# openai/jukebox

Measured on NVIDIA H100. Metric: top_prior_tokens_per_sec, higher is better.
Workload: dtype fp16

## Files before the change

### jukebox_b200/csrc/decode_engine.cu

```cuda
#include "engine.cuh"
#include <cooperative_groups.h>
#include <vector>
#include <algorithm>
#include <string.h>
#include <stdlib.h>
#include <math.h>

using namespace jk;

#ifndef JK_MMA_ALL_WARPS
#define JK_MMA_ALL_WARPS 1
#endif
#ifndef JK_QKV_POLL_BATCH
#define JK_QKV_POLL_BATCH 1
#endif
#ifndef JK_SKIP_FOREIGN_WAIT
#define JK_SKIP_FOREIGN_WAIT 1
#endif
#ifndef JK_LOGITS_MMA
#define JK_LOGITS_MMA 1
#endif
#ifndef JK_ATTN_LL_MERGE
#define JK_ATTN_LL_MERGE 1
#endif

namespace {

constexpr int kConsumers = 256;
constexpr int kThreads = 384;
constexpr int kSlotBytes = 16384;
constexpr int kMaxSlots = 12;
constexpr int kHeaderBytes = 8192;
constexpr int kLogitKT = 1024;
constexpr int kLogitRowsPerChunk = 4;
constexpr int kLogitRowsPerPass = 16;
constexpr int kMaxSplit = 4;
constexpr int kProfSlots = 1024;
// ... 31 lines not shown
    int slot;
    uint32_t phase;
    __device__ __forceinline__ static int nslot() { return sm_E()->nslot; }
    __device__ __forceinline__ uint64_t* full() const { return sm_full() + slot; }
    __device__ __forceinline__ uint64_t* empty() const { return sm_empty() + slot; }
    __device__ __forceinline__ uint8_t* data() const {
        const EngineDev* E = sm_E();
        return jk_smem + kHeaderBytes + E->uni_bytes + E->kvpre_bytes + slot * kSlotBytes;
    }
    __device__ __forceinline__ void advance() {
        if (++slot == nslot()) { slot = 0; phase ^= 1u; }
    }
};

#define STAMP(E_, slot_, i_)                                                                \
    do {                                                                                    \
        if (blockIdx.x == 0 && threadIdx.x == 0 && (E_)->prof_on && (slot_) < kProfSlots)      \
            (E_)->prof2[(size_t)(slot_) * 8 + (i_)] = clock64();                             \
    } while (0)

__device__ __forceinline__ void consumer_sync() { asm volatile("bar.sync 1, 256;" ::: "memory"); }

__device__ __host__ __forceinline__ int kpc_of(int ncg) { return ncg == 1 ? 64 : ncg == 2 ? 32 : ncg <= 4 ? 16 : 8; }

#define JK_ST_LL "st.relaxed.gpu.global"
__device__ __forceinline__ void ll_st(unsigned long long* p, uint32_t data, uint32_t flag) {
    const unsigned long long v = ((unsigned long long)flag << 32) | data;
    asm volatile(JK_ST_LL ".u64 [%0], %1;" ::"l"(p), "l"(v) : "memory");
}
__device__ __forceinline__ ulonglong2 ll_ld2(const unsigned long long* p) {
    ulonglong2 v;
    asm volatile("ld.relaxed.gpu.global.v2.u64 {%0,%1}, [%2];" : "=l"(v.x), "=l"(v.y) : "l"(p) : "memory");
    return v;
}
__device__ __forceinline__ unsigned long long ll_ld1(const unsigned long long* p) {
    unsigned long long v;
    asm volatile("ld.relaxed.gpu.global.u64 %0, [%1];" : "=l"(v) : "l"(p) : "memory");
    return v;
}
__constant__ int jk_nowait;
__device__ __forceinline__ bool ll_ok(unsigned long long w, uint32_t flag) { return ((uint32_t)(w >> 32) == flag) | (jk_nowait != 0); }
__device__ __forceinline__ void spin_guard(unsigned& spins) {
    if (++spins > (1u << 24)) __trap();
}
__device__ __forceinline__ uint32_t ll_wait1(const unsigned long long* p, uint32_t flag) {
    unsigned spins = 0;
    unsigned long long w = ll_ld1(p);
    while (!ll_ok(w, flag)) { spin_guard(spins); w = ll_ld1(p); }
    return (uint32_t)w;
}
__device__ __forceinline__ unsigned long long wait_stat_word(const long long* p, int G) {
    unsigned spins = 0;
    unsigned long long w = ll_ld1(reinterpret_cast<const unsigned long long*>(p));
    while ((int)(w >> kCntShift) != G && !jk_nowait) { spin_guard(spins); w = ll_ld1(reinterpret_cast<const unsigned long long*>(p)); }
    return w;
}

__device__ __forceinline__ float quick_gelu_f(float x) {
    const float z = h2f_round(1.702f * x);
    const float s = h2f_round(1.0f / (1.0f + expf(-z)));
    return x * s;
}

__device__ __forceinline__ long long fx_sum(float x) { return __float2ll_rn(x * 65536.0f); }
__device__ __forceinline__ long long fx_sq(float x) { return __float2ll_rn(fminf(x * x, 16777216.0f) * 16384.0f); }
__device__ __forceinline__ void red_add_u64(long long* p, unsigned long long v) {
    atomicAdd(reinterpret_cast<unsigned long long*>(p), v);
}
__device__ __forceinline__ long long* sm_sfx() { return reinterpret_cast<long long*>(sm_uni() + kRedBytes); }

__device__ __forceinline__ void publish_stats(long long* ln_out, int B, int ppc) {
    const int tid = threadIdx.x;
// ... 167 lines not shown

struct LogitsRec {
    float* lg_out;
    long long lg_bs;
    const float* lb;
    long long lb_bs;
    unsigned long long* xp;
    ushort2 cols;
};
__device__ __forceinline__ LogitsRec* sm_lrec() { return reinterpret_cast<LogitsRec*>(jk_smem + 7744); }

__device__ __noinline__ Ring gemm_phase(Ring ring, int B, int epi_, int l, int pslot_, uint32_t fl) {
    const EngineDev* E = sm_E();
    GemmArgs g;
    {
        const LayerDev& LD = *sm_layer(l);
        const ushort2* cl = reinterpret_cast<const ushort2*>(jk_smem + 1024 + 256 * (l & 1) + 128);
        const int W = E->W, S = E->S, M = E->M;
        long long* lnb = E->lnacc + (size_t)(2 * l) * 512;
        g.epi = epi_; g.pslot = pslot_; g.flag_in = fl; g.flag_out = fl;
        g.gamma = nullptr; g.beta = nullptr; g.ln_in = nullptr; g.ln_out = nullptr; g.ln = 0;
        g.lg_out = nullptr; g.lg_bs = 0; g.lb = nullptr; g.lb_bs = 0;
        if (epi_ == EPI_QKV) {
            g.in = E->ll_h; g.out = E->ll_qkv; g.xp = E->xp[0]; g.K = W; g.N = (LD.attn_func == 6) ? S : 3 * S;
            g.g0 = cl[0].x; g.ncg = cl[0].y; g.ln = 1; g.gamma = LD.ln0_g; g.beta = LD.ln0_b; g.bias = LD.b_qkv;
            g.ln_in = lnb; g.kind = 0; g.kin = W;
        } else if (epi_ == EPI_PROJ) {
            g.in = E->ll_a; g.out = E->ll_x1; g.xp = E->xp[1]; g.K = S; g.N = W; g.g0 = cl[1].x; g.ncg = cl[1].y;
            g.bias = LD.b_o; g.ln_out = lnb + 512; g.kind = 1; g.kin = S;
        } else if (epi_ == EPI_FC) {
            g.in = E->ll_x1; g.out = E->ll_g; g.xp = E->xp[2]; g.K = W; g.N = M; g.g0 = cl[2].x; g.ncg = cl[2].y;
            g.ln = 1; g.gamma = LD.ln1_g; g.beta = LD.ln1_b; g.bias = LD.b_1; g.ln_in = lnb + 512; g.kind = 0; g.kin = W;
        } else if (epi_ == EPI_PROJ2) {
            g.in = E->ll_g; g.out = E->ll_h; g.xp = E->xp[3]; g.K = M; g.N = W; g.g0 = cl[3].x; g.ncg = cl[3].y;
            g.bias = LD.b_2; g.ln_out = lnb + 1024; g.flag_out = fl + 1; g.kind = 2; g.kin = M;
        } else {
            const LogitsRec* lr = sm_lrec();
            g.in = E->ll_h; g.out = nullptr; g.xp = lr->xp; g.K = 2 * W; g.N = E->bins; g.g0 = lr->cols.x; g.ncg = lr->cols.y;
            g.bias = nullptr; g.kind = 2; g.kin = W; g.flag_out = 0;
            g.lg_out = lr->lg_out; g.lg_bs = lr->lg_bs; g.lb = lr->lb; g.lb_bs = lr->lb_bs;
        }
    }
    uint8_t* uni = sm_uni();
    const int tid = threadIdx.x, warp = tid >> 5, lane = tid & 31;
    const int KS = E->KS, ksh = E->ks_shift, c = blockIdx.x, rank = c & (KS - 1);
    const int ncg = g.ncg, nc = ncg * 8;
    const int ppc = (nc >> 1) >> ksh;
    const bool residual = (g.epi == EPI_PROJ || g.epi == EPI_PROJ2);
// ... 67 lines not shown
    STAMP(E, g.pslot, 2);
#if JK_MMA_ALL_WARPS
    const int nwarp = in_order ? min(8, nslots_phase) : min(8, nkk);
#else
    const int nwarp = min(8, (nkk + kpc - 1) >> (31 - __clz(kpc)));
#endif
    float* red = reinterpret_cast<float*>(uni);
    const int ncp = ((nc + 31) & ~31) + 8;
    unsigned long long* xp_unit = g.xp + (size_t)(c - rank) * 16 * kXpCols;
    {
        consumer_sync();
        if (warp < nwarp) {
            const int r0 = lane >> 2, c0 = (lane & 3) * 2;
#pragma unroll
            for (int j = 0; j < 8; ++j) {
                if (j < ncg) {
                    float* d = red + (size_t)(warp * 16) * ncp + j * 8 + c0;
                    *reinterpret_cast<float2*>(d + r0 * ncp) = make_float2(acc[j][0], acc[j][1]);
                    *reinterpret_cast<float2*>(d + (r0 + 8) * ncp) = make_float2(acc[j][2], acc[j][3]);
                }
            }
        }
        consumer_sync();
        if (KS > 1 && lane < (nc >> 1)) {
#pragma unroll 1
            for (int b = warp; b < B; b += 8) {
                float s0 = 0.f, s1 = 0.f;
                for (int w = 0; w < nwarp; ++w) {
                    const float2 v = *reinterpret_cast<const float2*>(red + (size_t)(w * 16 + b) * ncp + 2 * lane);
                    s0 += v.x; s1 += v.y;
                }
                unsigned long long* dst = xp_unit + ((size_t)rank * 16 + b) * kXpCols + 2 * lane;
                const unsigned long long fl = (unsigned long long)g.flag_in << 32;
                asm volatile(JK_ST_LL ".v2.u64 [%0], {%1,%2};" ::"l"(dst), "l"(fl | __float_as_uint(s0)),
                             "l"(fl | __float_as_uint(s1)) : "memory");
            }
        }
    }
    STAMP(E, g.pslot, 3);
    float2* res = sm_res();
    long long* sfx = sm_sfx();
    const bool two_rows = ppc <= 16;
    const int pl = two_rows ? (lane & 15) : lane;
    const int b_first = two_rows ? 2 * warp + (lane >> 4) : warp, b_step = two_rows ? 16 : 8;
    if (pl < ppc) {
        const int pr = rank * ppc + pl;
        const int gc = g.g0 * 8 + 2 * pr;
        const float2 bias = g.bias ? *reinterpret_cast<const float2*>(g.bias + gc) : make_float2(0.f, 0.f);
#pragma unroll 1
        for (int b = b_first; b < B; b += b_step) {
            float s0 = 0.f, s1 = 0.f;
            if (KS == 1) {
                for (int w = 0; w < nwarp; ++w) {
                    const float2 v = *reinterpret_cast<const float2*>(red + (size_t)(w * 16 + b) * ncp + 2 * pr);
                    s0 += v.x; s1 += v.y;
                }
            } else {
                ulonglong2 v[4];
                unsigned spins = 0;
                bool again;
                do {
                    again = false;
#pragma unroll
                    for (int q = 0; q < 4; ++q)
                        if (q < KS) v[q] = ll_ld2(xp_unit + ((size_t)q * 16 + b) * kXpCols + 2 * pr);
#pragma unroll
                    for (int q = 0; q < 4; ++q)
                        if (q < KS) again |= !(ll_ok(v[q].x, g.flag_in) && ll_ok(v[q].y, g.flag_in));
                    if (again) spin_guard(spins);
                } while (again);
#pragma unroll
                for (int q = 0; q < 4; ++q)
                    if (q < KS) { s0 += __uint_as_float((uint32_t)v[q].x); s1 += __uint_as_float((uint32_t)v[q].y); }
            }
            if (epi == EPI_LOGITS) {
                float* lo_ = g.lg_out + (size_t)b * g.lg_bs + gc;
                const float* lb_ = g.lb ? g.lb + (size_t)b * g.lb_bs + gc : nullptr;
                if (gc < N) lo_[0] = s0 + (lb_ ? lb_[0] : 0.f);
                if (gc + 1 < N) lo_[1] = s1 + (lb_ ? lb_[1] : 0.f);
                continue;
            }
            const float y0 = h2f_round(s0 + bias.x), y1 = h2f_round(s1 + bias.y);
            __half2 o;
            if (epi == EPI_QKV) {
                o = __floats2half2_rn(y0, y1);
            } else if (epi == EPI_FC) {
                o = __floats2half2_rn(quick_gelu_f(y0), quick_gelu_f(y1));
            } else {
                const float2 base = res[b * 32 + pl];
                const float o0 = h2f_round(base.x + y0), o1 = h2f_round(base.y + y1);
                res[b * 32 + pl] = make_float2(o0, o1);
                o = __floats2half2_rn(o0, o1);
                sfx[b * 32 + pl] = fx_sum(o0) + fx_sum(o1);
                sfx[1024 + b * 32 + pl] = fx_sq(o0) + fx_sq(o1);
            }
            ll_st(g.out + (size_t)b * (N >> 1) + (gc >> 1), *reinterpret_cast<const uint32_t*>(&o), g.flag_out);
        }
    }
    STAMP(E, g.pslot, 4);
    if (residual) publish_stats(g.ln_out, B, ppc);
    else consumer_sync();
    return ring;
}

struct AttnGeom {
    int R;
    int base;
    int cur;
    int wrow;
// ... 108 lines not shown
#pragma unroll
        for (int q = 0; q < 4; ++q) {
            const bool on = q < ns;
            m[q] = on ? __ldcg(p0 + (size_t)q * st) : -INFINITY;
            l[q] = on ? __ldcg(p0 + (size_t)q * st + 1) : 0.f;
            v[q] = (on && d < dh) ? __ldcg(reinterpret_cast<const float2*>(p0 + (size_t)q * st + 2 + d)) : make_float2(0.f, 0.f);
        }
        float M = -INFINITY;
#pragma unroll
        for (int q = 0; q < 4; ++q) M = fmaxf(M, m[q]);
        float Lsum = 0.f, o0 = 0.f, o1 = 0.f;
#pragma unroll
        for (int q = 0; q < 4; ++q) {
            if (q < ns) {
                const float w = expf(m[q] - M);
                Lsum += l[q] * w; o0 += v[q].x * w; o1 += v[q].y * w;
            }
        }
        if (d < dh) attn_out_pair(E, b, h, d, o0 / Lsum, o1 / Lsum, flag);
    }
}

__device__ __noinline__ void attn_item(const LayerDev& LD_ref, int b, int h, int s, int ns,
                                       const AttnGeom G, int pslot, uint32_t flag, int pre) {
    const EngineDev* E = sm_E();
    uint8_t* uni = sm_uni();
    float* stats = sm_stats();
    const LayerDev LD = LD_ref;
    const int tid = threadIdx.x, lane = tid & 31, warp = tid >> 5;
    const int dh = E->dh, dhp = E->dh_pad, S = E->S;
    const int nvec = dhp >> 3, npair = dhp >> 4;
    const int swz = (nvec & 7) ? 0 : 7;
    const int RC = E->RC;
    const int tileB = RC * dhp * 2;
    const uint32_t regU = smem_u32(uni), regX = smem_u32(jk_smem + kHeaderBytes + E->uni_bytes);
    const uint32_t regA = pre ? regX : regU, regB = pre ? regU : regX;
    __half* qh = reinterpret_cast<__half*>(uni + 2 * tileB);
    __half* kn = qh + dhp;
    __half* vn = kn + dhp;
    float* sc = reinterpret_cast<float*>(uni + 2 * tileB + 3 * dhp * 2);
    const int qkv_words = ((LD.attn_func == 6) ? S : 3 * S) >> 1;
    const unsigned long long* qrow = E->ll_qkv + (size_t)b * qkv_words + ((h * dh) >> 1);
    const size_t cbase = ((size_t)(b * E->H + h)) * LD.rows;
    const bool last_part = (s == ns - 1);
    const int R = G.R;
    const int ncache = R - ((R > 0 && G.cur) ? 1 : 0);
    const int i0 = div_small(ncache * s, ns), i1 = div_small(ncache * (s + 1), ns);
    const __half* kbase = LD.kc + (cbase + G.base) * dhp;
    const __half* vbase = LD.vc + (cbase + G.base) * dhp;
    const int trows = RC - 1;
    const int ntiles = max(1, (i1 - i0 + trows - 1) / trows);

    auto issue_tile = [&](int ti) {
        const int r0 = i0 + ti * trows, nr = max(0, min(trows, i1 - r0));
        const uint32_t kd = (ti & 1) ? regB : regA, vd = kd + tileB;
        kv_copy_tile(kd, vd, kbase + (size_t)r0 * dhp, vbase + (size_t)r0 * dhp, nr, dhp, swz);
    };
    STAMP(E, pslot, 0);
    if (R > 0 && !pre) issue_tile(0);
    {
        const int hw = dhp >> 1, dw = dh >> 1;
        const int nsel = (LD.attn_func == 6) ? 1 : 3;
#if JK_QKV_POLL_BATCH
        const int total = nsel * hw;
        unsigned long long wv[3];
        const unsigned long long* wp[3];
#pragma unroll
        for (int j = 0; j < 3; ++j) {
            const int i = tid + j * kConsumers;
            const int sel = (i >= hw) + (i >= 2 * hw), wd = i - sel * hw;
            wp[j] = (i < total && wd < dw) ? qrow + (size_t)sel * (S >> 1) + wd : nullptr;
            if (wp[j]) wv[j] = ll_ld1(wp[j]);
        }
        unsigned spins = 0;
        for (;;) {
            bool again = false;
#pragma unroll
            for (int j = 0; j < 3; ++j)
                if (wp[j] && !ll_ok(wv[j], flag)) { wv[j] = ll_ld1(wp[j]); again = true; }
            if (!again) break;
            spin_guard(spins);
        }
#pragma unroll
        for (int j = 0; j < 3; ++j) {
            const int i = tid + j * kConsumers;
            if (i < total) reinterpret_cast<uint32_t*>(qh)[i] = wp[j] ? (uint32_t)wv[j] : 0u;
        }
#else
        for (int i = tid; i < nsel * hw; i += kConsumers) {
            const int sel = i / hw, wd = i - sel * hw;
            uint32_t v = 0u;
            if (wd < dw) v = ll_wait1(qrow + (size_t)sel * (S >> 1) + wd, flag);
            reinterpret_cast<uint32_t*>(qh)[sel * hw + wd] = v;
        }
#endif
    }
    consumer_sync();
    if (G.wrow >= 0 && last_part) {
        for (int i = tid; i < dh; i += kConsumers) {
            LD.kc[(cbase + G.wrow) * dhp + i] = kn[i];
            LD.vc[(cbase + G.wrow) * dhp + i] = vn[i];
        }
    }
    if (R == 0) {
        if (2 * tid < dh) attn_out_pair(E, b, h, 2 * tid, 0.f, 0.f, flag);
        return;
    }

    float m_run = -INFINITY, l_run = 0.f;
    float* osm = sc + 64;
    const uint32_t qh_s = smem_u32(qh);
#pragma unroll 1
    for (int ti = 0; ti < ntiles; ++ti) {
        if (ti + 1 < ntiles) {
            issue_tile(ti + 1);
            asm volatile("cp.async.wait_group 1;" ::: "memory");
        } else {
            asm volatile("cp.async.wait_group 0;" ::: "memory");
// ... 151 lines not shown
            attn_out_pair(E, b, h, d, o0 / Lsum, o1 / Lsum, flag);
        }
        STAMP(E, pslot, 6);
        return;
    }
#endif
    const int item = b * E->H + h;
    if (tid == 0) {
        float* part = E->part + ((size_t)(item * kMaxSplit + s)) * (dhp + 2);
        part[0] = m_run; part[1] = l_run;
    }
    consumer_sync();
    if (tid == 0) {
        unsigned ticket;
        asm volatile("atom.acq_rel.gpu.global.add.u32 %0, [%1], 1;" : "=r"(ticket) : "l"(E->acnt + item) : "memory");
        stats[48] = (ticket == (unsigned)(ns - 1)) ? 1.f : 0.f;
        if (ticket == (unsigned)(ns - 1)) E->acnt[item] = 0u;
    }
    consumer_sync();
    if (stats[48] != 0.f) attn_merge(item, ns, b, h, flag);
    STAMP(E, pslot, 6);
}

__device__ __noinline__ int attn_prefetch(const LayerDev& LD_ref, int B, int c, int t, int pm, int pd, int gmax) {
    const EngineDev* E = sm_E();
    if (!E->kv_prefetch) return 0;
    const LayerDev LD = LD_ref;
    const AttnGeom G = attn_geom(E, LD, t, pm, pd);
    if (G.R == 0) return 0;
    const int ncache = G.R - (G.cur ? 1 : 0);
    const int ns = attn_nsplit(E, gmax, ncache);
    if (c >= B * E->H * ns) return 0;
    const int bh = div_small(c, ns), s = c - bh * ns, b = bh / E->H, h = bh - b * E->H;
    const int dhp = E->dh_pad, nvec = dhp >> 3, RC = E->RC;
    const int swz = (nvec & 7) ? 0 : 7;
    const int i0 = div_small(ncache * s, ns), i1 = div_small(ncache * (s + 1), ns);
    const int nr = max(0, min(RC - 1, i1 - i0));
    const size_t cbase = ((size_t)(b * E->H + h)) * LD.rows;
    const uint32_t kd = smem_u32(jk_smem + kHeaderBytes + E->uni_bytes), vd = kd + RC * dhp * 2;
    kv_copy_tile(kd, vd, LD.kc + (cbase + G.base + i0) * dhp, LD.vc + (cbase + G.base + i0) * dhp, nr, dhp, swz);
    return 1;
}

__device__ __noinline__ void producer_loop(const EngineDev* E, Ring ring, int do_logits, int c) {
    if ((threadIdx.x & 31) != 0) return;
    const uint8_t* src = E->streams + (size_t)c * E->stream_stride;
// ... 293 lines not shown
                const float2 pe = *reinterpret_cast<const float2*>(E->pos_emb + (size_t)launch_pos() * E->W + col);
                x.x += pe.x; x.y += pe.y;
                if (A.x_cond) {
                    const float2 xc = *reinterpret_cast<const float2*>(A.x_cond + ((size_t)b * A.x_cond_len + (A.x_cond_len > 1 ? launch_pos() : 0)) * E->W + col);
                    x.x += xc.x; x.y += xc.y;
                }
            }
            const __half2 hh = __floats2half2_rn(x.x, x.y);
            const float2 hv = __half22float2(hh);
            res[b * 32 + pl] = hv;
            sfx[b * 32 + pl] = fx_sum(hv.x) + fx_sum(hv.y);
            sfx[1024 + b * 32 + pl] = fx_sq(hv.x) + fx_sq(hv.y);
            ll_st(E->ll_h + (((size_t)b * E->W + col) >> 1), *reinterpret_cast<const uint32_t*>(&hh), launch_fbase() + 1);
        }
        publish_stats(LN_BLOCK(0), B, ppc);
    }
    PHASE_DONE();

#pragma unroll 1
    for (int l = 0; l < E->depth; ++l) {
        const LayerDev& LD = *sm_layer(l);
        const uint32_t fl = launch_fbase() + (uint32_t)l + 1;
        const int pre = attn_prefetch(LD, B, c, launch_pos(), PM, PD, GMAX);
        if (l == 1) PROF3(0, 0);
        ring = gemm_phase(ring, B, EPI_QKV, l, (int)nph, fl);
        if (l == 1) PROF3(0, 1);
        if (l > 0) CLEAR_AFTER(2 * l - 1, 2 * l);
        if (l + 1 < E->depth) {
#if JK_ASYNC_RECORD
            if (tid < (int)(sizeof(LayerDev) / 4))
                asm volatile("cp.async.ca.shared.global [%0], [%1], 4;" ::"r"(smem_u32(jk_smem + 1024 + 256 * ((l + 1) & 1) + 4 * tid)),
                             "l"(reinterpret_cast<const uint32_t*>(&Eg->layer[l + 1]) + tid) : "memory");
            if (tid >= 32 && tid < 36)
                asm volatile("cp.async.ca.shared.global [%0], [%1], 4;" ::"r"(smem_u32(jk_smem + 1024 + 256 * ((l + 1) & 1) + 128 + 4 * (tid - 32))),
                             "l"(reinterpret_cast<const uint32_t*>(E->cols + ((size_t)cta_unit() * E->depth + l + 1) * 4) + (tid - 32)) : "memory");
            asm volatile("cp.async.commit_group;" ::: "memory");
#else
            if (tid < (int)(sizeof(LayerDev) / 4))
                reinterpret_cast<uint32_t*>(jk_smem + 1024 + 256 * ((l + 1) & 1))[tid] =
                    reinterpret_cast<const uint32_t*>(&Eg->layer[l + 1])[tid];
            if (tid >= 32 && tid < 36)
                reinterpret_cast<uint32_t*>(jk_smem + 1024 + 256 * ((l + 1) & 1) + 128)[tid - 32] =
                    reinterpret_cast<const uint32_t*>(E->cols + ((size_t)cta_unit() * E->depth + l + 1) * 4)[tid - 32];
#endif
        }
        PHASE_DONE();
        if (l == 1) PROF3(1, 0);
        {
            const AttnGeom geo = attn_geom(E, LD, launch_pos(), PM, PD);
            const int ns = attn_nsplit(E, GMAX, geo.R - ((geo.R > 0 && geo.cur) ? 1 : 0));
            for (int it = c; it < B * E->H * ns; it += E->G) {
                const int bh = div_small(it, ns), s = it - bh * ns, ib = bh / E->H;
                attn_item(LD, ib, bh - ib * E->H, s, ns, geo, (int)nph, fl, pre && it == c);
                consumer_sync();
            }
        }
        if (l == 1) PROF3(1, 1);
        PHASE_DONE();
        if (l == 1) PROF3(2, 0);
        ring = gemm_phase(ring, B, EPI_PROJ, l, (int)nph, fl);
        if (l == 1) PROF3(2, 1);
        PHASE_DONE();
        if (l == 1) PROF3(3, 0);
        ring = gemm_phase(ring, B, EPI_FC, l, (int)nph, fl);
        if (l == 1) PROF3(3, 1);
        CLEAR_AFTER(2 * l, 2 * l + 1);
        PHASE_DONE();
        if (l == 1) PROF3(4, 0);
#if JK_ASYNC_RECORD
        asm volatile("cp.async.wait_group 0;" ::: "memory");
#endif
        ring = gemm_phase(ring, B, EPI_PROJ2, l, (int)nph, fl);
        if (l == 1) PROF3(4, 1);
        PHASE_DONE();
    }
    if (A.h_out) {
// ... 136 lines not shown
    for (int i = threadIdx.y; i < 32; i += blockDim.y) {
        const int n = n0 + i, k = k0 + threadIdx.x;
        if (n < N && k < K) dst[(size_t)n * K + k] = tile[threadIdx.x][i];
    }
}

__global__ void enc_kv_scatter_kernel(const __half* __restrict__ y, __half* kc, __half* vc, int rows_total, int E_dims,
                                      int S, int H, int dh, int dhp) {
    const size_t i = (size_t)blockIdx.x * blockDim.x + threadIdx.x;
    if (i >= (size_t)rows_total * 2 * S) return;
    const int r = (int)(i / (2 * S)), cidx = (int)(i % (2 * S));
    const int b = r / E_dims, e = r % E_dims;
    const int which = cidx / S, cs = cidx % S;
    const int h = cs / dh, d = cs % dh;
    __half* dst = which ? vc : kc;
    dst[(((size_t)(b * H + h)) * E_dims + e) * dhp + d] = y[i];
}

}

namespace {

struct Layout {
    size_t off_dev, off_cols, off_goff, off_lrow, off_streams, off_small, off_cache, off_h, off_x1, off_qkv, off_a, off_g, off_xp[4], off_part, off_acnt, off_prof, off_prof2, off_prof3, off_lnacc, off_encx, off_ency, off_wt, off_pf, off_sync, total;
    int KS, U;
    size_t wt_per_layer;
    int pf_len, pf_rows;
    size_t stream_stride;
    std::vector<ushort2> cols;
    std::vector<uint32_t> goff;
    std::vector<int> lrow;
    int lg_on, lg_np;
    std::vector<size_t> cache_off;
    std::vector<size_t> cache_bytes;
    std::vector<int> cache_rows;
    size_t small_per_layer;
    int dh, dh_pad, bc, prime_pad, uni_bytes, kvpre_bytes, kv_prefetch, nslot, smem_bytes, RC;
};

inline size_t align_up(size_t v, size_t a) { return (v + a - 1) / a * a; }

int cache_rows_for(const jk_prior_config& c, int af, int bc, int prime_pad) {
    switch (af) {
        case 0: return c.n_ctx;
        case 1: return bc;
        case 2: return c.n_ctx;
        case 3: return 2 * bc;
        case 6: return c.encoder_dims;
        case 7: return prime_pad;
    }
    return -1;
}

int compute_layout(const jk_prior_config& c, int G, Layout& L) {
// ... 42 lines not shown
            JK_REQUIRE(base + (extra ? 1 : 0) <= 8, "n_out %d too wide for %d units (max 64 columns per unit)", Ns[gi], U);
            std::vector<int> n(U, base);
            if (gi == 1 || gi == 3) {
                for (int i = 0; i < extra; ++i) n[i] += 1;
            } else {
                const unsigned long long chunk = (unsigned long long)(Ks[gi] / KS / 16) * 256ull;
                for (int i = 0; i < extra; ++i) {
                    int best = -1;
                    for (int u = 0; u < U; ++u)
                        if (n[u] < 8 && (best < 0 || cum[u] + n[u] * chunk < cum[best] + n[best] * chunk)) best = u;
                    n[best] += 1;
                }
            }
            int g0 = 0;
            for (int u = 0; u < U; ++u) {
                L.cols[((size_t)u * depth + l) * 4 + gi] = make_ushort2((unsigned short)g0, (unsigned short)n[u]);
                for (int r = 0; r < KS; ++r)
                    L.goff[((size_t)(u * KS + r) * depth + l) * 4 + gi] = (uint32_t)(cum[u] / 16);
                cum[u] += (unsigned long long)n[u] * (Ks[gi] / KS / 16) * 256ull;
                g0 += n[u];
            }
        }
    }
    L.lg_on = 0; L.lg_np = 0;
    {
        const int groups = (c.bins + 7) / 8;
        const int Kp = 2 * c.width;
        const int np = ((groups + U - 1) / U + 7) / 8;
        const bool ok = c.bins > 0 && KS >= 2 && (Kp / 16) % KS == 0 && c.width % (Kp / KS) == 0 &&
                        (size_t)16 * (Kp / KS + 8) * 2 <= (size_t)65536 && np <= 4 && !getenv("JK_NO_LOGITS_MMA");
        if (ok) {
            L.lg_on = 1; L.lg_np = np;
            L.cols.resize((size_t)U * depth * 4 + (size_t)np * U, make_ushort2(0, 0));
            L.goff.resize((size_t)G * depth * 4 + (size_t)np * G, 0);
            const int base = groups / U, extra = groups % U;
            std::vector<int> n(U, base);
            for (int i = 0; i < U; ++i) order[i] = i;
            std::stable_sort(order.begin(), order.end(), [&](int a, int b) { return cum[a] < cum[b]; });
            for (int i = 0; i < extra; ++i) n[order[i]] += 1;
            std::vector<int> g0(U, 0);
            for (int u = 1; u < U; ++u) g0[u] = g0[u - 1] + n[u - 1];
            for (int p = 0; p < np; ++p) {
                for (int u = 0; u < U; ++u) {
                    const int k = std::max(0, std::min(8, n[u] - 8 * p));
                    L.cols[(size_t)U * depth * 4 + (size_t)p * U + u] = make_ushort2((unsigned short)(g0[u] + 8 * p), (unsigned short)k);
                    for (int r = 0; r < KS; ++r) L.goff[(size_t)G * depth * 4 + (size_t)p * G + u * KS + r] = (uint32_t)(cum[u] / 16);
// ... 18 lines not shown
        uni = std::max(uni, (size_t)16 * kLogitKT * 4);
        uni = std::max(uni, (size_t)kRedBytes + 2 * 1024 * 8);
        const size_t kv_stage = (size_t)2 * RC * L.dh_pad * 2;
        size_t attn = kv_stage + (size_t)3 * L.dh_pad * 2 + 64 * 4 + (size_t)L.dh_pad * 4 + 64;
        uni = std::max(uni, attn);
        L.uni_bytes = (int)align_up(uni, 1024);
        L.kvpre_bytes = (int)align_up(kv_stage, 1024);
        nslot = (max_smem - kHeaderBytes - L.uni_bytes - L.kvpre_bytes) / kSlotBytes;
        if (nslot >= 4 || RC <= 16) break;
    }
    L.RC = RC;
    L.kv_prefetch = 0;
    nslot = std::min(nslot, kMaxSlots);
    JK_REQUIRE(nslot >= 2, "not enough shared memory for the weight ring (uni %d bytes)", L.uni_bytes);
    L.nslot = nslot;
    L.smem_bytes = kHeaderBytes + L.uni_bytes + L.kvpre_bytes + nslot * kSlotBytes;
    JK_REQUIRE((size_t)kHeaderBytes + (size_t)16 * (Kmax + 8) * 2 <= (size_t)L.smem_bytes, "A tile exceeds shared memory");

    size_t off = 0;
    L.off_dev = off; off = align_up(off + sizeof(EngineDev), 256);
    L.off_cols = off; off = align_up(off + L.cols.size() * sizeof(ushort2), 256);
    L.off_goff = off; off = align_up(off + L.goff.size() * 4, 256);
    L.off_lrow = off; off = align_up(off + L.lrow.size() * 4, 256);
    L.off_streams = off; off = align_up(off + (size_t)G * L.stream_stride, 256);
    L.small_per_layer = align_up((size_t)(3 * c.n_state + c.width + c.mlp_width + c.width + 4 * c.width) * 4, 256);
    L.off_small = off; off += L.small_per_layer * depth;
    for (int l = 0; l < depth; ++l)
        if (c.attn_func[l] == 6) off = align_up(off + (size_t)c.width * 2 * c.n_state * 2 + 2 * c.n_state * 4 + 512, 256);
    L.off_cache = off;
    L.cache_off.resize(depth); L.cache_bytes.resize(depth); L.cache_rows.resize(depth);
    for (int l = 0; l < depth; ++l) {
        int rows = cache_rows_for(c, c.attn_func[l], L.bc, L.prime_pad);
        L.cache_rows[l] = rows;
        size_t bytes = align_up((size_t)c.max_batch * c.heads * rows * L.dh_pad * 2, 256);
        L.cache_off[l] = off; L.cache_bytes[l] = bytes;
        off += 2 * bytes;
    }
    L.off_h = off;   off = align_up(off + (size_t)16 * c.width * 4, 256);
    L.off_x1 = off;  off = align_up(off + (size_t)16 * c.width * 4, 256);
    L.off_qkv = off; off = align_up(off + (size_t)16 * 3 * c.n_state * 4, 256);
    L.off_a = off;   off = align_up(off + (size_t)16 * c.n_state * 4, 256);
    L.off_g = off;   off = align_up(off + (size_t)16 * c.mlp_width * 4, 256);
    for (int gi = 0; gi < 4; ++gi) { L.off_xp[gi] = off; off = align_up(off + (size_t)G * 16 * kXpCols * 8, 256); }
    L.off_part = off; off = align_up(off + (size_t)c.max_batch * c.heads * kMaxSplit * (L.dh_pad + 2) * 8, 256);
    L.off_acnt = off; off = align_up(off + (size_t)c.max_batch * c.heads * 4, 256);
    L.off_prof = off; off = align_up(off + (size_t)kProfSlots * 8, 256);
    L.off_prof2 = off; off = align_up(off + (size_t)kProfSlots * 8 * 8, 256);
    L.off_prof3 = off; off = align_up(off + (size_t)5 * 256 * 2 * 8, 256);
    L.off_lnacc = off; off = align_up(off + (size_t)(2 * depth + 1) * 512 * 8, 256);
    {
        bool any6 = false;
        for (int l = 0; l < depth; ++l) any6 = any6 || (c.attn_func[l] == 6);
        L.off_encx = off; if (any6) off = align_up(off + (size_t)c.max_batch * c.encoder_dims * c.width * 2, 1024);
        L.off_ency = off; if (any6) off = align_up(off + (size_t)c.max_batch * c.encoder_dims * 2 * c.n_state * 2, 1024);
    }
    {
        auto k_ok = [](int k) { return k >= 64 && k % 8 == 0; };
        const bool ok = k_ok(c.width) && k_ok(c.n_state) && k_ok(c.mlp_width) && !getenv("JK_NO_PREFILL");
        int cap = c.n_ctx;
        if (const char* e = getenv("JK_PREFILL_MAX")) cap = std::max(2, std::min(cap, atoi(e)));
        L.pf_len = ok ? cap : 0;
        L.pf_rows = c.max_batch * L.pf_len;
        L.wt_per_layer = align_up((size_t)(3 * c.n_state * c.width + c.width * c.n_state + 2 * c.mlp_width * c.width) * 2, 1024);
// ... 75 lines not shown
    E.W = cfg->width; E.S = cfg->n_state; E.M = cfg->mlp_width; E.H = cfg->heads; E.dh = L.dh; E.dh_pad = L.dh_pad;
    E.L = cfg->n_ctx; E.blocks = cfg->blocks; E.bc = L.bc; E.bins = cfg->bins; E.prime_pad = L.prime_pad;
    E.enc_dims = cfg->encoder_dims; E.Bmax = cfg->max_batch; E.add_cond_after = cfg->add_cond_after;
    E.depth = cfg->depth; E.G = G; E.KS = L.KS; E.ks_shift = L.KS == 4 ? 2 : L.KS == 2 ? 1 : 0; E.U = L.U; E.RC = L.RC; E.nslot = L.nslot; E.uni_bytes = L.uni_bytes; E.kvpre_bytes = L.kvpre_bytes; E.small_bytes = (int)L.small_per_layer; E.prof_on = getenv("JK_PROFILE") ? 1 : 0;
    E.kv_prefetch = getenv("JK_KV_PREFETCH") ? atoi(getenv("JK_KV_PREFETCH")) : 1;
    {
        const int nowait = getenv("JK_NOWAIT") ? atoi(getenv("JK_NOWAIT")) : 0;
        JK_CHECK_CUDA(cudaMemcpyToSymbol(jk_nowait, &nowait, sizeof(int)));
    }
    {
        double sc = 1.0 / sqrt(sqrt((double)L.dh));
        E.scale2 = (float)(sc * sc);
    }
    E.cols = (const ushort2*)(A + L.off_cols);
    p->d_cols = (ushort2*)(A + L.off_cols);
    p->d_goff = (uint32_t*)(A + L.off_goff);
    E.lrow0 = (const int*)(A + L.off_lrow);
    E.lg_on = L.lg_on; p->lg_on = L.lg_on;
    E.lg_np = L.lg_np; p->lg_np = L.lg_np;
    E.lg_cols = (const ushort2*)(A + L.off_cols) + (size_t)L.U * cfg->depth * 4;
    E.lg_goff = (const uint32_t*)(A + L.off_goff) + (size_t)G * cfg->depth * 4;
    E.streams = A + L.off_streams; E.stream_stride = L.stream_stride;
    E.ll_h = (unsigned long long*)(A + L.off_h); E.ll_x1 = (unsigned long long*)(A + L.off_x1);
    E.ll_qkv = (unsigned long long*)(A + L.off_qkv); E.ll_a = (unsigned long long*)(A + L.off_a);
    E.ll_g = (unsigned long long*)(A + L.off_g);
    for (int gi = 0; gi < 4; ++gi) E.xp[gi] = (unsigned long long*)(A + L.off_xp[gi]);
    E.part = (float*)(A + L.off_part);
    E.acnt = (unsigned*)(A + L.off_acnt); E.prof = (unsigned long long*)(A + L.off_prof);
    E.lnacc = (long long*)(A + L.off_lnacc);
    E.prof2 = (long long*)(A + L.off_prof2);
    E.prof3 = (unsigned long long*)(A + L.off_prof3);
    E.sync = (unsigned*)(A + L.off_sync); E.t = (int*)(E.sync + 96);
    size_t enc_off = L.off_small + L.small_per_layer * cfg->depth;
    for (int i = 0; i < 4; ++i) { p->bias_ptr[i].resize(cfg->depth); p->ln_ptr[i].resize(cfg->depth); }
    p->enc_w.assign(cfg->depth, nullptr); p->enc_b.assign(cfg->depth, nullptr);
    for (int l = 0; l < cfg->depth; ++l) {
        LayerDev& LD = E.layer[l];
        LD.attn_func = cfg->attn_func[l];
        LD.rows = L.cache_rows[l];
        LD.kc = (__half*)(A + L.cache_off[l]);
        LD.vc = (__half*)(A + L.cache_off[l] + L.cache_bytes[l]);
        float* s = (float*)(A + L.off_small + L.small_per_layer * l);
        p->bias_ptr[0][l] = s; s += 3 * cfg->n_state;
        p->bias_ptr[1][l] = s; s += cfg->width;
        p->bias_ptr[2][l] = s; s += cfg->mlp_width;
        p->bias_ptr[3][l] = s; s += cfg->width;
        for (int i = 0; i < 4; ++i) { p->ln_ptr[i][l] = s; s += cfg->width; }
// ... 14 lines not shown
    p->pf_rows = L.pf_rows; p->pf_len = L.pf_len;
    for (int i = 0; i < 4; ++i) p->wt[i].assign(cfg->depth, nullptr);
    if (L.pf_rows) {
        for (int l = 0; l < cfg->depth; ++l) {
            __half* w = (__half*)(A + L.off_wt + L.wt_per_layer * l);
            p->wt[0][l] = w; w += (size_t)3 * cfg->n_state * cfg->width;
            p->wt[1][l] = w; w += (size_t)cfg->width * cfg->n_state;
            p->wt[2][l] = w; w += (size_t)cfg->mlp_width * cfg->width;
            p->wt[3][l] = w;
        }
        __half* a = (__half*)(A + L.off_pf);
        const size_t R = (size_t)L.pf_rows;
        p->pf_x = a; a += R * cfg->width;
        p->pf_xn = a; a += R * cfg->width;
        p->pf_x1 = a; a += R * cfg->width;
        p->pf_qkv = a; a += R * 3 * cfg->n_state;
        p->pf_a = a; a += R * cfg->n_state;
        p->pf_g = a;
    }
    p->dev = (EngineDev*)(A + L.off_dev);
    JK_CHECK_CUDA(cudaMemcpyAsync(A + L.off_cols, L.cols.data(), L.cols.size() * sizeof(ushort2), cudaMemcpyHostToDevice, stream));
    JK_CHECK_CUDA(cudaMemcpyAsync(A + L.off_goff, L.goff.data(), L.goff.size() * 4, cudaMemcpyHostToDevice, stream));
    JK_CHECK_CUDA(cudaMemcpyAsync(A + L.off_lrow, L.lrow.data(), L.lrow.size() * 4, cudaMemcpyHostToDevice, stream));
    JK_CHECK_CUDA(cudaMemcpyAsync(p->dev, &p->host, sizeof(EngineDev), cudaMemcpyHostToDevice, stream));
    JK_CHECK_CUDA(cudaStreamSynchronize(stream));
    {
        int dev = 0, optin = 0;
        JK_CHECK_CUDA(cudaGetDevice(&dev));
        JK_CHECK_CUDA(cudaDeviceGetAttribute(&optin, cudaDevAttrMaxSharedMemoryPerBlockOptin, dev));
        JK_REQUIRE(L.smem_bytes <= optin, "decode kernel needs %d bytes of shared memory, device allows %d", L.smem_bytes, optin);
        JK_CHECK_CUDA(cudaFuncSetAttribute(jk_decode_step_kernel, cudaFuncAttributeMaxDynamicSharedMemorySize, optin));
    }
    *out = p;
    return 0;
}

extern "C" int jk_prior_destroy(jk_prior* p) {
    delete p;
    return 0;
}

template <typename T>
static int pack_one(jk_prior* p, const void* w, int K, int N, int l, int gi, cudaStream_t stream) {
    pack_gemm_kernel<T><<<p->G, 256, 0, stream>>>((const T*)w, K, N, (uint8_t*)p->host.streams, p->host.stream_stride,
                                                   p->d_cols, p->d_goff, p->cfg.depth, l, gi, p->host.KS);
    JK_CHECK_CUDA(cudaGetLastError());
// ... 150 lines not shown
```

### jukebox_b200/csrc/engine.cuh

```cuda
#pragma once
#include "common.cuh"
#include "../../include/jkb200.h"
#include <vector>

namespace jk {

struct LayerDev {
    int attn_func;
    int rows;
    __half* kc;
    __half* vc;
    const float *ln0_g, *ln0_b, *ln1_g, *ln1_b;
    const float *b_qkv, *b_o, *b_1, *b_2;
    const __half* enc_w;
    const float* enc_b;
};

struct EngineDev {
    int W, S, M, H, dh, dh_pad, L, blocks, bc, bins, prime_pad, enc_dims, Bmax, add_cond_after, depth, G;
    int RC;
    int ks_shift;
    int KS, U;
    int nslot, uni_bytes, kvpre_bytes, small_bytes, prof_on, kv_prefetch;
    float scale2;
    const ushort2* cols;
    const uint8_t* streams;
    unsigned long long stream_stride;
    unsigned long long *ll_h, *ll_x1, *ll_qkv, *ll_a, *ll_g;
    unsigned long long* xp[4];
    float* part;
    unsigned* acnt;
    long long* lnacc;
    long long* prof2;
    unsigned long long* prof3;
    unsigned long long* prof;
    unsigned* sync;
    int* t;
    const float *x_emb, *pos_emb, *x_out, *start_token;
    const int* lrow0;
    int lg_on, lg_np;
    const ushort2* lg_cols;
    const uint32_t* lg_goff;
    LayerDev layer[JK_MAX_DEPTH];
};

int gemm_f16_tc(const void* x, const void* w_t, const float* bias, const void* res, void* y, int M, int N, int K,
                int epi, cudaStream_t stream);

}

struct jk_prior {
    jk_prior_config cfg;
// ... 23 lines not shown
```

Before: 7289.

## Fuse QKV epilogue into attention by reading split-K partials directly

The QKV GEMM no longer runs its epilogue or publishes the ll_qkv buffer. Instead, attention items read the per-unit split-K partial products through a precomputed column-to-unit map, sum them, add the bias and round to fp16 themselves. Non-final splits fetch only q. The map is prefetched into shared memory with cp.async before the GEMM phase. This removes one publish/poll hop and the epilogue pass on the critical path, at the cost of more polling loads per attention thread (up to four partials per word) and more complex wait-group bookkeeping.

```diff
diff --git a/jukebox_b200/csrc/decode_engine.cu b/jukebox_b200/csrc/decode_engine.cu
--- a/jukebox_b200/csrc/decode_engine.cu
+++ b/jukebox_b200/csrc/decode_engine.cu
@@ -10,9 +10,6 @@
 
 #ifndef JK_MMA_ALL_WARPS
 #define JK_MMA_ALL_WARPS 1
-#endif
-#ifndef JK_QKV_POLL_BATCH
-#define JK_QKV_POLL_BATCH 1
 #endif
 #ifndef JK_SKIP_FOREIGN_WAIT
 #define JK_SKIP_FOREIGN_WAIT 1
@@ -90,6 +87,8 @@
 __device__ __forceinline__ void consumer_sync() { asm volatile("bar.sync 1, 256;" ::: "memory"); }
 
 __device__ __host__ __forceinline__ int kpc_of(int ncg) { return ncg == 1 ? 64 : ncg == 2 ? 32 : ncg <= 4 ? 16 : 8; }
+constexpr int kQmapSmem = 1536;
+constexpr int kQmapSel = 68;
 
 #define JK_ST_LL "st.relaxed.gpu.global"
 __device__ __forceinline__ void ll_st(unsigned long long* p, uint32_t data, uint32_t flag) {
@@ -110,12 +109,6 @@
 __device__ __forceinline__ bool ll_ok(unsigned long long w, uint32_t flag) { return ((uint32_t)(w >> 32) == flag) | (jk_nowait != 0); }
 __device__ __forceinline__ void spin_guard(unsigned& spins) {
     if (++spins > (1u << 24)) __trap();
-}
-__device__ __forceinline__ uint32_t ll_wait1(const unsigned long long* p, uint32_t flag) {
-    unsigned spins = 0;
-    unsigned long long w = ll_ld1(p);
-    while (!ll_ok(w, flag)) { spin_guard(spins); w = ll_ld1(p); }
-    return (uint32_t)w;
 }
 __device__ __forceinline__ unsigned long long wait_stat_word(const long long* p, int G) {
     unsigned spins = 0;
@@ -329,8 +322,8 @@
         g.gamma = nullptr; g.beta = nullptr; g.ln_in = nullptr; g.ln_out = nullptr; g.ln = 0;
         g.lg_out = nullptr; g.lg_bs = 0; g.lb = nullptr; g.lb_bs = 0;
         if (epi_ == EPI_QKV) {
-            g.in = E->ll_h; g.out = E->ll_qkv; g.xp = E->xp[0]; g.K = W; g.N = (LD.attn_func == 6) ? S : 3 * S;
-            g.g0 = cl[0].x; g.ncg = cl[0].y; g.ln = 1; g.gamma = LD.ln0_g; g.beta = LD.ln0_b; g.bias = LD.b_qkv;
+            g.in = E->ll_h; g.out = nullptr; g.xp = E->xp[0]; g.K = W; g.N = (LD.attn_func == 6) ? S : 3 * S;
+            g.g0 = cl[0].x; g.ncg = cl[0].y; g.ln = 1; g.gamma = LD.ln0_g; g.beta = LD.ln0_b; g.bias = nullptr;
             g.ln_in = lnb; g.kind = 0; g.kin = W;
         } else if (epi_ == EPI_PROJ) {
             g.in = E->ll_a; g.out = E->ll_x1; g.xp = E->xp[1]; g.K = S; g.N = W; g.g0 = cl[1].x; g.ncg = cl[1].y;
@@ -444,7 +437,7 @@
             }
         }
         consumer_sync();
-        if (KS > 1 && lane < (nc >> 1)) {
+        if ((KS > 1 || epi == EPI_QKV) && lane < (nc >> 1)) {
 #pragma unroll 1
             for (int b = warp; b < B; b += 8) {
                 float s0 = 0.f, s1 = 0.f;
@@ -460,6 +453,11 @@
         }
     }
     STAMP(E, g.pslot, 3);
+    if (epi == EPI_QKV) {
+        consumer_sync();
+        STAMP(E, g.pslot, 4);
+        return ring;
+    }
     float2* res = sm_res();
     long long* sfx = sm_sfx();
     const bool two_rows = ppc <= 16;
@@ -504,9 +502,7 @@
             }
             const float y0 = h2f_round(s0 + bias.x), y1 = h2f_round(s1 + bias.y);
             __half2 o;
-            if (epi == EPI_QKV) {
-                o = __floats2half2_rn(y0, y1);
-            } else if (epi == EPI_FC) {
+            if (epi == EPI_FC) {
                 o = __floats2half2_rn(quick_gelu_f(y0), quick_gelu_f(y1));
             } else {
                 const float2 base = res[b * 32 + pl];
@@ -661,11 +657,12 @@
 }
 
 __device__ __noinline__ void attn_item(const LayerDev& LD_ref, int b, int h, int s, int ns,
-                                       const AttnGeom G, int pslot, uint32_t flag, int pre) {
+                                       const AttnGeom G, int pslot, uint32_t flag, int pre_younger) {
     const EngineDev* E = sm_E();
     uint8_t* uni = sm_uni();
     float* stats = sm_stats();
     const LayerDev LD = LD_ref;
+    const int pre = pre_younger & 1, younger = pre_younger >> 1;
     const int tid = threadIdx.x, lane = tid & 31, warp = tid >> 5;
     const int dh = E->dh, dhp = E->dh_pad, S = E->S;
     const int nvec = dhp >> 3, npair = dhp >> 4;
@@ -678,8 +675,6 @@
     __half* kn = qh + dhp;
     __half* vn = kn + dhp;
     float* sc = reinterpret_cast<float*>(uni + 2 * tileB + 3 * dhp * 2);
-    const int qkv_words = ((LD.attn_func == 6) ? S : 3 * S) >> 1;
-    const unsigned long long* qrow = E->ll_qkv + (size_t)b * qkv_words + ((h * dh) >> 1);
     const size_t cbase = ((size_t)(b * E->H + h)) * LD.rows;
     const bool last_part = (s == ns - 1);
     const int R = G.R;
@@ -698,41 +693,67 @@
     STAMP(E, pslot, 0);
     if (R > 0 && !pre) issue_tile(0);
     {
+        const int yg = younger + ((R > 0 && !pre) ? 1 : 0);
+        if (yg == 0) asm volatile("cp.async.wait_group 0;" ::: "memory");
+        else if (yg == 1) asm volatile("cp.async.wait_group 1;" ::: "memory");
+        else asm volatile("cp.async.wait_group 2;" ::: "memory");
+        consumer_sync();
         const int hw = dhp >> 1, dw = dh >> 1;
-        const int nsel = (LD.attn_func == 6) ? 1 : 3;
-#if JK_QKV_POLL_BATCH
-        const int total = nsel * hw;
-        unsigned long long wv[3];
-        const unsigned long long* wp[3];
-#pragma unroll
-        for (int j = 0; j < 3; ++j) {
-            const int i = tid + j * kConsumers;
-            const int sel = (i >= hw) + (i >= 2 * hw), wd = i - sel * hw;
-            wp[j] = (i < total && wd < dw) ? qrow + (size_t)sel * (S >> 1) + wd : nullptr;
-            if (wp[j]) wv[j] = ll_ld1(wp[j]);
-        }
-        unsigned spins = 0;
-        for (;;) {
-            bool again = false;
-#pragma unroll
-            for (int j = 0; j < 3; ++j)
-                if (wp[j] && !ll_ok(wv[j], flag)) { wv[j] = ll_ld1(wp[j]); again = true; }
-            if (!again) break;
-            spin_guard(spins);
-        }
-#pragma unroll
-        for (int j = 0; j < 3; ++j) {
-            const int i = tid + j * kConsumers;
-            if (i < total) reinterpret_cast<uint32_t*>(qh)[i] = wp[j] ? (uint32_t)wv[j] : 0u;
-        }
-#else
-        for (int i = tid; i < nsel * hw; i += kConsumers) {
-            const int sel = i / hw, wd = i - sel * hw;
-            uint32_t v = 0u;
-            if (wd < dw) v = ll_wait1(qrow + (size_t)sel * (S >> 1) + wd, flag);
-            reinterpret_cast<uint32_t*>(qh)[sel * hw + wd] = v;
-        }
-#endif
+        const int nsel = (LD.attn_func == 6 || !last_part) ? 1 : 3;
+        const int total = nsel * hw, KS = E->KS;
+        const uint16_t* qm = reinterpret_cast<const uint16_t*>(jk_smem + kQmapSmem);
+        const unsigned long long* xp0 = E->xp[0];
+#pragma unroll 1
+        for (int i0 = tid; i0 < total; i0 += 2 * kConsumers) {
+            ulonglong2 pv[2][4];
+            float2 bias[2];
+            int wo[2];
+            bool act[2];
+#pragma unroll
+            for (int j = 0; j < 2; ++j) {
+                const int i = i0 + j * kConsumers;
+                const int sel = (i >= hw) + (i >= 2 * hw), wd = i - sel * hw;
+                const int c0 = sel * S + h * dh, col = c0 + 2 * wd;
+                act[j] = i < total && wd < dw;
+                const unsigned e = act[j] ? qm[sel * kQmapSel + (col >> 3) - ((c0 >> 3) & ~1)] : 0u;
+                wo[j] = act[j] ? ((int)(e >> 3) * KS * 16 + b) * kXpCols + (e & 7) * 8 + (col & 7) : 0;
+                bias[j] = *reinterpret_cast<const float2*>(LD.b_qkv + (act[j] ? col : 0));
+#pragma unroll
+                for (int q = 0; q < 4; ++q) pv[j][q] = ll_ld2(xp0 + wo[j] + min(q, KS - 1) * 16 * kXpCols);
+            }
+            unsigned spins = 0;
+            for (;;) {
+                bool again = false;
+#pragma unroll
+                for (int j = 0; j < 2; ++j) {
+#pragma unroll
+                    for (int q = 0; q < 4; ++q) {
+                        if (act[j] && !(ll_ok(pv[j][q].x, flag) && ll_ok(pv[j][q].y, flag))) {
+                            pv[j][q] = ll_ld2(xp0 + wo[j] + min(q, KS - 1) * 16 * kXpCols);
+                            again = true;
+                        }
+                    }
+                }
+                if (!again) break;
+                spin_guard(spins);
+            }
+#pragma unroll
+            for (int j = 0; j < 2; ++j) {
+                const int i = i0 + j * kConsumers;
+                if (i < total) {
+                    uint32_t word = 0u;
+                    if (act[j]) {
+                        float s0 = 0.f, s1 = 0.f;
+#pragma unroll
+                        for (int q = 0; q < 4; ++q)
+                            if (q < KS) { s0 += __uint_as_float((uint32_t)pv[j][q].x); s1 += __uint_as_float((uint32_t)pv[j][q].y); }
+                        const __half2 o = __floats2half2_rn(h2f_round(s0 + bias[j].x), h2f_round(s1 + bias[j].y));
+                        word = *reinterpret_cast<const uint32_t*>(&o);
+                    }
+                    reinterpret_cast<uint32_t*>(qh)[i] = word;
+                }
+            }
+        }
     }
     consumer_sync();
     if (G.wrow >= 0 && last_part) {
@@ -930,6 +951,20 @@
     STAMP(E, pslot, 6);
 }
 
+__device__ __noinline__ void qkv_map_fetch(int l, int h) {
+    const EngineDev* E = sm_E();
+    const int tid = threadIdx.x, S = E->S, dh = E->dh;
+    const int sel = tid / (kQmapSel / 2), wi = tid - sel * (kQmapSel / 2);
+    if (sel < ((sm_layer(l)->attn_func == 6) ? 1 : 3)) {
+        const int c0 = sel * S + h * dh;
+        const int glo = (c0 >> 3) & ~1, ghi = (c0 + dh - 1) >> 3;
+        if (glo + 2 * wi <= ghi)
+            asm volatile("cp.async.ca.shared.global [%0], [%1], 4;" ::"r"(smem_u32(jk_smem + kQmapSmem + sel * kQmapSel * 2 + 4 * wi)),
+                         "l"(E->qmap + (size_t)l * ((3 * S) >> 3) + glo + 2 * wi) : "memory");
+    }
+    asm volatile("cp.async.commit_group;" ::: "memory");
+}
+
 __device__ __noinline__ int attn_prefetch(const LayerDev& LD_ref, int B, int c, int t, int pm, int pd, int gmax) {
     const EngineDev* E = sm_E();
     if (!E->kv_prefetch) return 0;
@@ -1269,6 +1304,11 @@
         const LayerDev& LD = *sm_layer(l);
         const uint32_t fl = launch_fbase() + (uint32_t)l + 1;
         const int pre = attn_prefetch(LD, B, c, launch_pos(), PM, PD, GMAX);
+        {
+            const AttnGeom geo = attn_geom(E, LD, launch_pos(), PM, PD);
+            const int ns = attn_nsplit(E, GMAX, geo.R - ((geo.R > 0 && geo.cur) ? 1 : 0));
+            if (c < B * E->H * ns) { const int bh = div_small(c, ns); qkv_map_fetch(l, bh - (bh / E->H) * E->H); }
+        }
         if (l == 1) PROF3(0, 0);
         ring = gemm_phase(ring, B, EPI_QKV, l, (int)nph, fl);
         if (l == 1) PROF3(0, 1);
@@ -1298,7 +1338,9 @@
             const int ns = attn_nsplit(E, GMAX, geo.R - ((geo.R > 0 && geo.cur) ? 1 : 0));
             for (int it = c; it < B * E->H * ns; it += E->G) {
                 const int bh = div_small(it, ns), s = it - bh * ns, ib = bh / E->H;
-                attn_item(LD, ib, bh - ib * E->H, s, ns, geo, (int)nph, fl, pre && it == c);
+                if (it != c) qkv_map_fetch(l, bh - ib * E->H);
+                const int younger = (JK_ASYNC_RECORD && it == c && l + 1 < E->depth) ? 1 : 0;
+                attn_item(LD, ib, bh - ib * E->H, s, ns, geo, (int)nph, fl, (pre && it == c) | younger << 1);
                 consumer_sync();
             }
         }
@@ -1481,7 +1523,7 @@
 namespace {
 
 struct Layout {
-    size_t off_dev, off_cols, off_goff, off_lrow, off_streams, off_small, off_cache, off_h, off_x1, off_qkv, off_a, off_g, off_xp[4], off_part, off_acnt, off_prof, off_prof2, off_prof3, off_lnacc, off_encx, off_ency, off_wt, off_pf, off_sync, total;
+    size_t off_dev, off_cols, off_goff, off_lrow, off_qmap, off_streams, off_small, off_cache, off_h, off_x1, off_a, off_g, off_xp[4], off_part, off_acnt, off_prof, off_prof2, off_prof3, off_lnacc, off_encx, off_ency, off_wt, off_pf, off_sync, total;
     int KS, U;
     size_t wt_per_layer;
     int pf_len, pf_rows;
@@ -1489,6 +1531,7 @@
     std::vector<ushort2> cols;
     std::vector<uint32_t> goff;
     std::vector<int> lrow;
+    std::vector<uint16_t> qmap;
     int lg_on, lg_np;
     std::vector<size_t> cache_off;
     std::vector<size_t> cache_bytes;
@@ -1577,6 +1620,16 @@
             }
         }
     }
+    {
+        const size_t qs = (size_t)3 * c.n_state / 8;
+        L.qmap.assign(qs * depth + 2, 0);
+        JK_REQUIRE(U < 8192, "too many units for the q / k / v column map");
+        for (int l = 0; l < depth; ++l)
+            for (int u = 0; u < U; ++u) {
+                const ushort2 cg = L.cols[((size_t)u * depth + l) * 4];
+                for (int j = 0; j < cg.y; ++j) L.qmap[qs * l + cg.x + j] = (uint16_t)(u << 3 | j);
+            }
+    }
     L.lg_on = 0; L.lg_np = 0;
     {
         const int groups = (c.bins + 7) / 8;
@@ -1641,6 +1694,7 @@
     L.off_cols = off; off = align_up(off + L.cols.size() * sizeof(ushort2), 256);
     L.off_goff = off; off = align_up(off + L.goff.size() * 4, 256);
     L.off_lrow = off; off = align_up(off + L.lrow.size() * 4, 256);
+    L.off_qmap = off; off = align_up(off + L.qmap.size() * 2, 256);
     L.off_streams = off; off = align_up(off + (size_t)G * L.stream_stride, 256);
     L.small_per_layer = align_up((size_t)(3 * c.n_state + c.width + c.mlp_width + c.width + 4 * c.width) * 4, 256);
     L.off_small = off; off += L.small_per_layer * depth;
@@ -1657,7 +1711,6 @@
     }
     L.off_h = off;   off = align_up(off + (size_t)16 * c.width * 4, 256);
     L.off_x1 = off;  off = align_up(off + (size_t)16 * c.width * 4, 256);
-    L.off_qkv = off; off = align_up(off + (size_t)16 * 3 * c.n_state * 4, 256);
     L.off_a = off;   off = align_up(off + (size_t)16 * c.n_state * 4, 256);
     L.off_g = off;   off = align_up(off + (size_t)16 * c.mlp_width * 4, 256);
     for (int gi = 0; gi < 4; ++gi) { L.off_xp[gi] = off; off = align_up(off + (size_t)G * 16 * kXpCols * 8, 256); }
@@ -1779,7 +1832,8 @@
     E.lg_goff = (const uint32_t*)(A + L.off_goff) + (size_t)G * cfg->depth * 4;
     E.streams = A + L.off_streams; E.stream_stride = L.stream_stride;
     E.ll_h = (unsigned long long*)(A + L.off_h); E.ll_x1 = (unsigned long long*)(A + L.off_x1);
-    E.ll_qkv = (unsigned long long*)(A + L.off_qkv); E.ll_a = (unsigned long long*)(A + L.off_a);
+    E.ll_a = (unsigned long long*)(A + L.off_a);
+    E.qmap = (const uint16_t*)(A + L.off_qmap);
     E.ll_g = (unsigned long long*)(A + L.off_g);
     for (int gi = 0; gi < 4; ++gi) E.xp[gi] = (unsigned long long*)(A + L.off_xp[gi]);
     E.part = (float*)(A + L.off_part);
@@ -1840,6 +1894,7 @@
     JK_CHECK_CUDA(cudaMemcpyAsync(A + L.off_cols, L.cols.data(), L.cols.size() * sizeof(ushort2), cudaMemcpyHostToDevice, stream));
     JK_CHECK_CUDA(cudaMemcpyAsync(A + L.off_goff, L.goff.data(), L.goff.size() * 4, cudaMemcpyHostToDevice, stream));
     JK_CHECK_CUDA(cudaMemcpyAsync(A + L.off_lrow, L.lrow.data(), L.lrow.size() * 4, cudaMemcpyHostToDevice, stream));
+    JK_CHECK_CUDA(cudaMemcpyAsync(A + L.off_qmap, L.qmap.data(), L.qmap.size() * 2, cudaMemcpyHostToDevice, stream));
     JK_CHECK_CUDA(cudaMemcpyAsync(p->dev, &p->host, sizeof(EngineDev), cudaMemcpyHostToDevice, stream));
     JK_CHECK_CUDA(cudaStreamSynchronize(stream));
     {
diff --git a/jukebox_b200/csrc/engine.cuh b/jukebox_b200/csrc/engine.cuh
--- a/jukebox_b200/csrc/engine.cuh
+++ b/jukebox_b200/csrc/engine.cuh
@@ -26,8 +26,9 @@
     const ushort2* cols;
     const uint8_t* streams;
     unsigned long long stream_stride;
-    unsigned long long *ll_h, *ll_x1, *ll_qkv, *ll_a, *ll_g;
+    unsigned long long *ll_h, *ll_x1, *ll_a, *ll_g;
     unsigned long long* xp[4];
+    const uint16_t* qmap;
     float* part;
     unsigned* acnt;
     long long* lnacc;
```

After: 7485 (median of 6 runs). 1.03x the previous value.
